# gfxdisp/ColorVideoVDP

Measured on AMD Instinct MI355X. Metric: Mpixels/s, higher is better.
Workload: dtype f32; 1 GPU; 3840x2160 60fps, standard_4k, f32 input resident in HBM, 64-frame clip pair; frames_total=64, frames_this_gpu=64, input_dtype=f32, heatmap=none, frame_generator=cpu, block_frames=64, fused_levels=3

## Files before the change

### colorvideovdp_amd/_capi.py

```python
import ctypes as C
import os

MAX_FILTER_LEN = 65
MAX_LEVELS = 16
MAX_WINDOW = 256
CSF_NODES = 32
PROF_N = 6
PROF_NAMES = ("photometry", "temporal_fir", "pyr_reduce", "band_level0", "band_rest", "heatmap")
ABI_VERSION = 14
RESIZE_MODES = {"nearest": 0, "bilinear": 1, "bicubic": 2, "area": 3}

U8, U16, F16, F32, F32_DKL, YUV8, YUV16 = range(7)
HEATMAP = {None: 0, "none": 0, "raw": 1, "threshold": 2, "supra-threshold": 3}
BUF_HIST, BUF_GPYR, BUF_DDUMP, BUF_HEAT, BUF_Q, BUF_HSTATS, BUF_HCURVE = range(7)


class Params(C.Structure):
    _fields_ = [
        ("eotf", C.c_int32),
        ("Y_peak", C.c_float), ("Y_black", C.c_float), ("Y_refl", C.c_float), ("exposure", C.c_float),
        ("gamma", C.c_float),
        ("rgb2dkl", C.c_float * 9),
        ("mask_p", C.c_float),
        ("mask_c10", C.c_float),
        ("mask_q", C.c_float * 4),
        ("xcm", C.c_float * 16),
        ("ch_gain", C.c_float * 4),
        ("d_max10", C.c_float),
        ("sens_mul", C.c_float),
        ("blur_radius", C.c_int32),
        ("blur_taps", C.c_float * 13),
        ("beta", C.c_float), ("beta_t", C.c_float), ("beta_tch", C.c_float), ("beta_sch", C.c_float),
        ("jod_a", C.c_float), ("jod_exp", C.c_float), ("image_int", C.c_float),
        ("ch_w", C.c_float * 4),
        ("baseband_weight", C.c_float * 4),
        ("csf_logL_first", C.c_float), ("csf_logL_last", C.c_float),
    ]


class Clip(C.Structure):
    _fields_ = [
        ("batch", C.c_int32), ("channels", C.c_int32),
        ("height", C.c_int32), ("width", C.c_int32),
        ("is_video", C.c_int32),
        ("n_frames", C.c_int32),
        ("first_frame", C.c_int32),
        ("n_levels", C.c_int32),
        ("filter_len", C.c_int32),
        ("block_frames", C.c_int32),
        ("heatmap", C.c_int32),
        ("debug_dump", C.c_int32),
        ("raw_halo", C.c_int32), ("total_frames", C.c_int32),
        ("feature_size", C.c_int32), ("fuse_mode", C.c_int32), ("band_layout", C.c_int32),
        ("defer_bands", C.c_int32), ("score_frames", C.c_int32),
        ("taps", C.c_float * (4 * MAX_FILTER_LEN)),
        ("csf_rows", C.c_float * (MAX_LEVELS * 4 * CSF_NODES)),
    ]


class YuvFormat(C.Structure):
    _fields_ = [
        ("chroma", C.c_int32), ("bit_depth", C.c_int32), ("matrix", C.c_int32), ("reserved", C.c_int32),
        ("frame_stride_test", C.c_int64), ("frame_stride_ref", C.c_int64),
    ]


PSNR_AS_IS, PSNR_PU21, PSNR_Y, PSNR_RGB2020 = range(4)


class PsnrArgs(C.Structure):
    _fields_ = [
        ("target", C.c_int32), ("reserved", C.c_int32),
        ("pu_p", C.c_float * 7),
        ("pu_L_min", C.c_float), ("pu_L_max", C.c_float),
        ("pu_norm", C.c_float),
        ("rows", C.c_float * 9),
    ]


SSIM_WIN = 11


class SsimArgs(C.Structure):
    _fields_ = [
        ("target", C.c_int32), ("reserved", C.c_int32),
        ("win", C.c_float * SSIM_WIN),
        ("C1", C.c_float), ("C2", C.c_float),
        ("luma", C.c_float * 3),
        ("pu_p", C.c_float * 7),
        ("pu_L_min", C.c_float), ("pu_L_max", C.c_float),
        ("pu_norm", C.c_float),
    ]


MSSSIM_LEVELS = 5


class MsssimArgs(C.Structure):
    _fields_ = [
        ("ssim", SsimArgs),
        ("weights", C.c_float * MSSSIM_LEVELS),
        ("reserved", C.c_int32),
    ]


PREVIEW_AS_IS, PREVIEW_LINEAR, PREVIEW_PQ = range(3)
PREVIEW_F32, PREVIEW_RGBE, PREVIEW_RGB48 = range(3)
# ... 156 lines not shown
```

### colorvideovdp_amd/csrc/core.cpp

```cpp
#include <algorithm>
#include <cmath>
#include <cstdarg>
#include <cstdio>
#include <cstdlib>
#include <cstring>
#include <string>
#include <vector>

#include "kernels.h"

using namespace cvvdp;

namespace {

struct Level {
  int H = 0, W = 0;
  int64_t P = 0;
  size_t g_off = 0, heat_off = 0, dd_off = 0, fd_off = 0, fs_off = 0;
  bool split_edge = false;
  bool feat4 = false;
  int f_pieces = 0;
  size_t partial_off = 0;
  int n_strip = 1, n_seg = 1, seg_h = 1;
  bool blur = false;
// ... 77 lines not shown
  return CVVDP_OK;
}

void join_pipeline(cvvdp_handle* h, hipStream_t s) {
  for (int i = 0; i < 2; ++i) {
    if (h->band_pending[i]) {
      (void)hipStreamWaitEvent(s, h->ev_band[i], 0);
      h->band_pending[i] = false;
    }
  }
}

struct ProfScope {
  cvvdp_handle* h; hipStream_t s; ProfEvent* ev = nullptr;
  ProfScope(cvvdp_handle* h_, int cat, hipStream_t s_) : h(h_), s(s_) {
    if (!h->prof) return;
    if (h->events_used == h->events.size()) {
      ProfEvent e{};
      if (hipEventCreate(&e.a) != hipSuccess || hipEventCreate(&e.b) != hipSuccess) return;
      h->events.push_back(e);
    }
    ev = &h->events[h->events_used++];
    ev->cat = cat;
    (void)hipEventRecord(ev->a, s);
  }
  ~ProfScope() { if (ev) (void)hipEventRecord(ev->b, s); }
};

constexpr float kGaussK0 = (float)(0.25 - 0.4 / 2.0);

void fill_csf(const cvvdp_handle* h, int level, float* lut) {
  std::memcpy(lut, h->c.csf_rows + (size_t)level * 4 * CVVDP_CSF_NODES, sizeof(float) * 4 * CVVDP_CSF_NODES);
}

void heat_weights(const cvvdp_handle* h, bool baseband, float* w) {
  const float t_int = h->c.is_video ? 1.0f : h->p.image_int;
  for (int c = 0; c < 4; ++c) {
    w[c] = h->p.ch_w[c] * t_int;
    if (baseband) w[c] = w[c] * h->p.baseband_weight[c];
  }
}

int run_bands(cvvdp_handle* h, int n_frames, int q_frame_offset, int set, hipStream_t s, int l_begin = 0, int l_end = -1, bool fused = false, int item0 = 0);

int run_pyramid_and_bands(cvvdp_handle* h, int n_frames, int q_frame_offset, hipStream_t s, int item0 = 0) {
  const int B = h->c.batch, items = n_frames * B, L = h->L, nch = h->nch;
  const float K[5] = {kGaussK0, 0.25f, 0.4f, 0.25f, kGaussK0};
  const int set = h->pipeline ? h->cur_set : 0;
  static const bool fuse2 = dev_knob("CVVDP_REDUCE2", 1) != 0;
  const int F = h->pipeline ? 0 : h->fuse_levels;
  if (F > 0) {
    if (int e = run_bands(h, n_frames, q_frame_offset, 0, s, 0, F, true, item0)) return e;
  }
  for (int l = F; l + 1 < L; ++l) {
    ProfScope ps(h, CVVDP_PROF_REDUCE, s);
    if (fuse2 && l + 2 < L && reduce2_supported(h->lv[l].H, h->lv[l].W)) {
      Reduce2Args r{};
      r.in = gbase(h, l, set) + (l == 0 ? (size_t)item0 * h->lv[0].P : 0); r.out1 = gbase(h, l + 1, set); r.out2 = gbase(h, l + 2, set);
      r.H = h->lv[l].H; r.W = h->lv[l].W; r.H1 = h->lv[l + 1].H; r.W1 = h->lv[l + 1].W; r.H2 = h->lv[l + 2].H; r.W2 = h->lv[l + 2].W;
      r.n_img = items; r.img_cap = level_cap(h, l); r.img_cap_out = h->items_cap_s; r.n_planes = 2 * nch;
      for (int i = 0; i < 5; ++i) r.k[i] = K[i];
      launch_reduce2(r, s);
      ++l;
      continue;
    }
    ReduceArgs r{};
    r.in = gbase(h, l, set) + (l == 0 ? (size_t)item0 * h->lv[0].P : 0);
    r.out = gbase(h, l + 1, set);
    r.H = h->lv[l].H; r.W = h->lv[l].W; r.Ho = h->lv[l + 1].H; r.Wo = h->lv[l + 1].W;
    r.n_img = items; r.img_cap = level_cap(h, l); r.img_cap_out = h->items_cap_s; r.n_planes = 2 * nch;
    for (int i = 0; i < 5; ++i) r.k[i] = K[i];
    launch_reduce(r, s);
  }
  if (int e = check_launch(h, "reduce")) return e;
  if (!h->pipeline) return run_bands(h, n_frames, q_frame_offset, 0, s, F, -1, false, item0);
  if (int e = ensure_pipeline_objects(h)) return e;
  (void)hipEventRecord(h->ev_reduce[set], s);
  (void)hipStreamWaitEvent(h->band_stream, h->ev_reduce[set], 0);
  if (int e = run_bands(h, n_frames, q_frame_offset, set, h->band_stream)) return e;
  (void)hipEventRecord(h->ev_band[set], h->band_stream);
  h->band_pending[set] = true;
  h->cur_set ^= 1;
  return CVVDP_OK;
}

int run_bands(cvvdp_handle* h, int n_frames, int q_frame_offset, int set, hipStream_t s, int l_begin, int l_end, bool fused, int item0) {
  const int B = h->c.batch, items = n_frames * B, L = h->L, nch = h->nch;
  if (l_begin == 0) h->last_range_done = false;
  if (l_end < 0) l_end = L - 1;
  const float K[5] = {kGaussK0, 0.25f, 0.4f, 0.25f, kGaussK0};
  const bool heat = h->c.heatmap != CVVDP_HEATMAP_NONE;
  static const bool fork_env = dev_knob("CVVDP_BAND_STREAMS", 1) != 0;
  static const int fork_max = dev_knob("CVVDP_BAND_STREAMS_MAX", 1024);
  static const int fork_tail = dev_knob("CVVDP_BAND_STREAMS_TAIL", 1);
  const int l_size = (fork_tail && !fused) ? std::min(l_begin, L - 1) : 0;
  bool fork = !fused && fork_env && L - l_size >= 4 && (int64_t)items * h->lv[l_size].n_strip * h->lv[l_size].n_seg <= fork_max;
  if (fork && !h->aux_stream[0]) {
    bool ok = hipEventCreateWithFlags(&h->ev_fork, hipEventDisableTiming) == hipSuccess;
    for (int i = 0; i < 2 && ok; ++i)
      ok = hipStreamCreateWithFlags(&h->aux_stream[i], hipStreamNonBlocking) == hipSuccess &&
           hipEventCreateWithFlags(&h->ev_join[i], hipEventDisableTiming) == hipSuccess;
    if (!ok) return fail(h, CVVDP_E_HIP, "cannot create the side streams of the band stage");
  }
  if (fork) {
    (void)hipEventRecord(h->ev_fork, s);
    for (int i = 0; i < 2; ++i) (void)hipStreamWaitEvent(h->aux_stream[i], h->ev_fork, 0);
  }
  hipStream_t const s_main = s;
// ... 160 lines not shown
    if (h->edge_stream[i]) { (void)hipStreamSynchronize(h->edge_stream[i]); (void)hipStreamDestroy(h->edge_stream[i]); }
    if (h->ev_edge_fork[i]) (void)hipEventDestroy(h->ev_edge_fork[i]);
    if (h->ev_edge_join[i]) (void)hipEventDestroy(h->ev_edge_join[i]);
  }
  delete h;
}

const char* cvvdp_last_error(const cvvdp_handle* h) { return h ? t_err.c_str() : "null handle"; }
int cvvdp_build_flags(void) {
  int f = tu_flags_band4() | tu_flags_band4f() | tu_flags_band4s();
#ifdef CVVDP_DEV_KNOBS
  f |= CVVDP_BUILD_DEV_KNOBS;
#endif
  return f;
}

#define CVVDP_STR2(x) #x
#define CVVDP_STR(x) CVVDP_STR2(x)
const char* cvvdp_build_info(void) {
#ifdef __clang_version__
#define CVVDP_COMPILER "clang " __clang_version__
#else
#define CVVDP_COMPILER "host compiler " __VERSION__
#endif
  return CVVDP_COMPILER "; HIP " CVVDP_STR(HIP_VERSION_MAJOR) "." CVVDP_STR(HIP_VERSION_MINOR) "." CVVDP_STR(HIP_VERSION_PATCH) "; gfx950";
}
int cvvdp_compiled_hip_version(void) { return HIP_VERSION; }
int cvvdp_runtime_hip_version(void) {
  int v = 0;
  if (hipRuntimeGetVersion(&v) != hipSuccess) return 0;
  return v;
}

int cvvdp_configure(cvvdp_handle* h, const cvvdp_clip* clip) {
  if (!h || !clip) return CVVDP_E_ARG;
  if (h->band_stream && (h->band_pending[0] || h->band_pending[1])) {
    (void)hipStreamSynchronize(h->band_stream);
    h->band_pending[0] = h->band_pending[1] = false;
  }
  const cvvdp_clip& c = *clip;
  if (c.batch < 1 || c.height < 2 || c.width < 2 || c.n_frames < 1) return fail(h, CVVDP_E_ARG, "bad clip geometry");
  if (c.channels != 1 && c.channels != 3) return fail(h, CVVDP_E_ARG, "channels must be 1 or 3");
  if (c.n_levels < 1 || c.n_levels > CVVDP_MAX_LEVELS) return fail(h, CVVDP_E_ARG, "n_levels out of range");
  if (c.is_video) {
    if (c.filter_len < 1 || c.filter_len > CVVDP_MAX_FILTER_LEN) return fail(h, CVVDP_E_UNSUPPORTED, "filter_len %d unsupported (max %d)", c.filter_len, CVVDP_MAX_FILTER_LEN);
    if (c.block_frames < 1 || c.filter_len - 1 + c.block_frames > CVVDP_MAX_WINDOW) return fail(h, CVVDP_E_ARG, "block_frames out of range");
  }
  if (c.heatmap != CVVDP_HEATMAP_NONE && c.batch != 1) return fail(h, CVVDP_E_UNSUPPORTED, "heat maps need batch == 1");
  if (c.feature_size < 0) return fail(h, CVVDP_E_ARG, "feature_size must be >= 0");
  if (c.feature_size > 0 && (c.heatmap != CVVDP_HEATMAP_NONE || c.debug_dump))
    return fail(h, CVVDP_E_UNSUPPORTED, "feature_size > 0 cannot be combined with a heat map or debug_dump");
  if (c.fuse_mode < 0 || c.fuse_mode > 2) return fail(h, CVVDP_E_ARG, "fuse_mode must be 0, 1 or 2");
  if (c.band_layout < 0 || c.band_layout > 1) return fail(h, CVVDP_E_ARG, "band_layout must be 0 or 1");
  if (c.defer_bands < 0 || c.defer_bands > 1) return fail(h, CVVDP_E_ARG, "defer_bands must be 0 or 1");
  if (c.defer_bands) {
    if (!c.is_video) return fail(h, CVVDP_E_ARG, "defer_bands is for video clips");
    if (c.score_frames < 1 || c.score_frames > c.block_frames) return fail(h, CVVDP_E_ARG, "score_frames must be in 1 .. block_frames");
    if (c.debug_dump || c.feature_size > 0) return fail(h, CVVDP_E_UNSUPPORTED, "defer_bands cannot be combined with debug_dump or features");
  }
  h->c = c;
  h->nch = c.is_video ? 4 : 3;
  h->L = c.n_levels;
  h->items_cap = (c.is_video ? c.block_frames : 1) * c.batch;
  h->items_cap_s = c.defer_bands ? c.score_frames * c.batch : h->items_cap;
  h->filtered_frames = 0;
  h->lv.assign(h->L, Level());
  int H = c.height, W = c.width;
  const int pad = h->p.blur_radius;
  for (int l = 0; l < h->L; ++l) {
    Level& lv = h->lv[l];
    lv.H = H; lv.W = W; lv.P = (int64_t)H * W;
    lv.blur = pad > 0 && H > pad && W > pad;
    lv.vec4 = lv.blur && W >= 16 && H >= 16;
    lv.feat4 = c.feature_size > 0 && lv.vec4 && l + 1 < h->L;
    const int sw = lv.vec4 ? kBand4StripWidth : (lv.blur ? 256 - 2 * pad : 256);
    lv.n_strip = (W + sw - 1) / sw;
    {
      const int clip_frames = c.total_frames > 0 ? c.total_frames : 64;
      static const int target_env = dev_knob("CVVDP_SEG_TARGET", 0);
      static const int rows_env = dev_knob("CVVDP_SEG_ROWS", 0);
      const int nominal = c.is_video ? std::min(c.heatmap != CVVDP_HEATMAP_NONE ? 16 : 64, clip_frames) : 1, target = target_env > 0 ? target_env : 768;
      const int max_rows = rows_env > 0 ? rows_env : (c.is_video ? 384 : 256);
      const int per_seg = lv.n_strip * nominal * c.batch;
      const int want = (target + per_seg - 1) / per_seg;
      const int lo = (H + max_rows - 1) / max_rows, hi = std::max(lo, (H + 15) / 16);
      lv.n_seg = std::min(std::max(want, lo), hi);
      lv.seg_h = (H + lv.n_seg - 1) / lv.n_seg;
      lv.seg_h += lv.seg_h & 1;
      lv.n_seg = (H + lv.seg_h - 1) / lv.seg_h;
      const int n_edge = lv.vec4 ? band4_edge_strips(W, lv.n_strip) : 0;
      lv.split_edge = n_edge > 0 && n_edge < lv.n_strip && (int64_t)(lv.n_strip - n_edge) * lv.n_seg * nominal * c.batch >= 1536;
    }
    if (l + 1 < h->L && (H < 2 || W < 2)) return fail(h, CVVDP_E_ARG, "pyramid too deep for %dx%d", c.width, c.height);
    H = (H + 1) / 2; W = (W + 1) / 2;
  }
  if (pad != 0 && pad != 6) return fail(h, CVVDP_E_UNSUPPORTED, "blur radius %d unsupported", pad);
  h->fuse_levels = 0;
  {
    const int clip_frames = c.total_frames > 0 ? c.total_frames : 64;
    const int nominal = c.is_video ? std::min(64, clip_frames) : 1;
    static const int fuse_max = dev_knob("CVVDP_FUSE_LEVELS", CVVDP_MAX_LEVELS);
    const bool plain = c.is_video && !c.debug_dump;
    const bool big = (int64_t)nominal * c.batch * h->lv[0].n_strip * h->lv[0].n_seg > 1024;
    if (plain && c.fuse_mode != 2 && (big || c.fuse_mode == 1))
      while (h->fuse_levels < fuse_max && h->fuse_levels + 1 < h->L && h->lv[h->fuse_levels].vec4 &&
             band4f_supported(h->lv[h->fuse_levels].H, h->lv[h->fuse_levels].W) &&
// ... 940 lines not shown
```

### colorvideovdp_amd/csrc/kernels.h

```cpp
#pragma once
#include <hip/hip_runtime.h>
#include <stdint.h>
#include "../../include/cvvdp_hip.h"

namespace cvvdp {

constexpr float kEps = 0.00001f;

#ifdef CVVDP_DEV_KNOBS
inline int dev_knob(const char* name, int dflt) { const char* v = getenv(name); return v ? atoi(v) : dflt; }
#else
constexpr int dev_knob(const char*, int dflt) { return dflt; }
#endif

#ifdef __HIPCC__
__device__ __forceinline__ float fast_log2(float x) { return __builtin_amdgcn_logf(x); }
__device__ __forceinline__ float fast_exp2(float x) { return __builtin_amdgcn_exp2f(x); }
__device__ __forceinline__ float fast_rcp(float x) { return __builtin_amdgcn_rcpf(x); }
__device__ __forceinline__ float fast_pow(float x, float p) { return fast_exp2(p * fast_log2(x)); }

__device__ __forceinline__ float expand_even(float m0, float m1, float m2, float e0, float e1) {
  return __builtin_fmaf(m2, e0, __builtin_fmaf(m1, e1, m0 * e0));
}
__device__ __forceinline__ float expand_odd(float m1, float m2, float eo) { return __builtin_fmaf(m2, eo, m1 * eo); }
// ... 56 lines not shown
void launch_resize(const ResizeArgs& a, hipStream_t s);
struct FirArgs {
  const void* src[2];
  int64_t sb[2], sc[2], sf[2], sh[2], sw[2];
  int32_t dtype;
  DisplayArgs dm;
  int32_t W, P, batch, n_frames, fl;
  int32_t raw_first;
  int32_t abs_first;
  int32_t write_hist;
  int32_t halo_run;
  float* hist;
  int64_t h_side, h_plane, h_slot, h_b;
  float* out;
  int64_t o_plane;
  float taps[4 * CVVDP_MAX_FILTER_LEN];
  float taps_rot[4 * CVVDP_ROT_TAPS];
  YuvArgs yuv;
  int16_t hist_src[CVVDP_MAX_FILTER_LEN];
};
static_assert(sizeof(FirArgs) <= 4096, "kernel arguments of the temporal kernels");
void launch_fir(const FirArgs& a, float* hist_shadow, hipStream_t s);
inline bool fir_has_register_window(int fl) { return fl == 7 || fl == 9 || fl == 13 || fl == 15 || fl == 17 || fl == 25 || fl == 31; }
inline int fir_kernel_len(int fl) {
  const int have[] = {7, 9, 13, 15, 17, 25, 31};
  for (int k : have) if (fl > 1 && fl <= k) return k;
  return fl;
}

struct ResampleArgs {
  FirArgs f;
  int32_t n_src[2];
  int32_t n_out, depth;
  const float* weights[2];
  const int32_t* emit[2];
  float* out[2];
};
static_assert(sizeof(ResampleArgs) <= 4096, "kernel arguments of the resampling temporal kernel");
inline bool fir_resampled_has_window(int depth) { return depth == 8 || depth == 12 || depth == 18 || depth == 26; }
void launch_fir_resampled(const ResampleArgs& a, bool generic, hipStream_t s);
int fir_resampled_prepare(cvvdp_handle* h, const void* t, const void* r, const cvvdp_yuv_format* fmt, int32_t H, int32_t W,
                          const int32_t n_src[2], int32_t depth, const float* w_t, const float* w_r, const int32_t* e_t, const int32_t* e_r,
                          int32_t n_out, float* out_t, float* out_r, ResampleArgs& a);
int fir_resampled_check_launch(cvvdp_handle* h);

struct ReduceArgs {
  const float* in;
  float* out;
  int32_t H, W, Ho, Wo, n_img;
  int32_t img_cap;
  int32_t img_cap_out;
  int32_t n_planes;
  float k[5];
};
void launch_reduce(const ReduceArgs& a, hipStream_t s);
struct Reduce2Args {
  const float* in;
  float *out1, *out2;
  int32_t H, W, H1, W1, H2, W2, n_img, img_cap, img_cap_out, n_planes;
  int32_t seg2;
  float k[5];
};
bool reduce2_supported(int H, int W);
constexpr int64_t kReduceRefPixels = 16384;
bool reduce_takes_ref_kernel(int H, int W);
void launch_reduce2(const Reduce2Args& a, hipStream_t s);

struct BandArgs {
  const float* g;
  const float* gc;
  int32_t H, W, Hc, Wc;
  int32_t items, items_cap, items_cap_c, nch;
  int32_t seg_h, n_seg, n_strip;
  int32_t per_xcd;
  int32_t strip0, n_strip_l;
  float band_mul;
  float lut[4 * CVVDP_CSF_NODES];
  float logL_first, logL_last;
  float sens_mul;
  float ch_gain[4];
  float mask_c10, mask_p, eps_p;
  float q[4], eps_q[4];
  float xw[16];
  float dmax;
  float m1[4];
  float inv_dmax;
  float blur_h[13];
  float ind_k1, ind_k0;
  float blur[13];
  float kx[3];
  float* partial;
  float* dchr;
  uint32_t* hstats;
  float hw[4];
  float beta_tch, eps_btch, eps_inv_btch;
  float* ddump;
  float* fdump;
  float* fsum;
  int32_t fs, f_pieces;
  float* g1_out;
  float rk[5];
  int32_t one_wave_layout;
};
void launch_band(const BandArgs& a, bool blur, hipStream_t s);
void launch_band4(const BandArgs& a, bool split_edge, hipStream_t s, hipStream_t s_edge);
int band4_edge_strips(int W, int n_strip);
// ... 395 lines not shown
```

### colorvideovdp_amd/csrc/pyramid.hip

```cpp
#include <algorithm>
#include <cstdlib>
#include <type_traits>
#include "kernels.h"

namespace cvvdp {

constexpr int RT = 32;
constexpr int RIN = 2 * RT + 3;

__device__ __forceinline__ float dot5(float a0, float a1, float a2, float a3, float a4, float k0, float k1, float k2, float k3, float k4) {
  return __builtin_fmaf(a4, k4, __builtin_fmaf(a3, k3, __builtin_fmaf(a2, k2, __builtin_fmaf(a1, k1, a0 * k0))));
}
__device__ __forceinline__ float dot2(float a0, float a1, float k0, float k1) { return __builtin_fmaf(a1, k1, a0 * k0); }
__device__ __forceinline__ float mul_rn(float a, float b) {
#pragma clang fp contract(off)
  return a * b;
}
__device__ __forceinline__ float add_rn(float a, float b) {
#pragma clang fp contract(off)
  return a + b;
}
__device__ __forceinline__ float edge2_rn(float v, float x0, float k0, float x1, float k1) { return add_rn(v, add_rn(mul_rn(x0, k0), mul_rn(x1, k1))); }

__global__ __launch_bounds__(256) void k_reduce(ReduceArgs a) {
  __shared__ float s_in[RIN][RIN + 1];
  __shared__ float s_v[RT][RIN + 1];
  const int img = blockIdx.z;
  const int plane = img / a.n_img, it = img - plane * a.n_img;
  const float* in = a.in + ((int64_t)plane * a.img_cap + it) * a.H * a.W;
  float* out = a.out + ((int64_t)plane * a.img_cap_out + it) * a.Ho * a.Wo;
  const int oy0 = blockIdx.y * RT, ox0 = blockIdx.x * RT;
  const int iy0 = 2 * oy0 - 2, ix0 = 2 * ox0 - 2;
  const int t = threadIdx.x;
  for (int e = t; e < RIN * RIN; e += 256) {
    const int r = e / RIN, c = e - r * RIN;
    const int y = iy0 + r, x = ix0 + c;
    s_in[r][c] = (y >= 0 && y < a.H && x >= 0 && x < a.W) ? in[(int64_t)y * a.W + x] : 0.0f;
  }
  __syncthreads();
  const float k0 = a.k[0], k1 = a.k[1], k2 = a.k[2], k3 = a.k[3], k4 = a.k[4];
  for (int e = t; e < RT * RIN; e += 256) {
    const int r = e / RIN, c = e - r * RIN;
    const int oy = oy0 + r;
    float v = 0.0f;
    if (oy < a.Ho && ix0 + c >= 0 && ix0 + c < a.W) {
      const int pr = 2 * r;
      v = dot5(s_in[pr][c], s_in[pr + 1][c], s_in[pr + 2][c], s_in[pr + 3][c], s_in[pr + 4][c], k0, k1, k2, k3, k4);
      if (oy == 0) v = edge2_rn(v, s_in[0 - iy0][c], k1, s_in[1 - iy0][c], k0);
      if (oy == a.Ho - 1) {
        if (a.H & 1) v = edge2_rn(v, s_in[a.H - 1 - iy0][c], k3, s_in[a.H - 2 - iy0][c], k4);
        else v = add_rn(v, mul_rn(s_in[a.H - 1 - iy0][c], k4));
      }
    }
    s_v[r][c] = v;
  }
  __syncthreads();
  for (int e = t; e < RT * RT; e += 256) {
    const int r = e / RT, c = e - r * RT;
    const int oy = oy0 + r, ox = ox0 + c;
    if (oy >= a.Ho || ox >= a.Wo) continue;
    const int pc = 2 * c;
    float v = dot5(s_v[r][pc], s_v[r][pc + 1], s_v[r][pc + 2], s_v[r][pc + 3], s_v[r][pc + 4], k0, k1, k2, k3, k4);
    if (ox == 0) v = edge2_rn(v, s_v[r][0 - ix0], k1, s_v[r][1 - ix0], k0);
    if (ox == a.Wo - 1) {
      if (a.H & 1) v = edge2_rn(v, s_v[r][a.W - 1 - ix0], k3, s_v[r][a.W - 2 - ix0], k4);
      else v = add_rn(v, mul_rn(s_v[r][a.W - 1 - ix0], k4));
    }
    out[(int64_t)oy * a.Wo + ox] = v;
  }
}

constexpr int RSEG = 32;
typedef float v4f_ __attribute__((ext_vector_type(4)));

template <bool EDGE>
__device__ __forceinline__ void hreduce_row(const ReduceArgs& a, const float* img, int y, float live, int ox, bool first, bool last, float (&h)[4]) {
  const int ix = 2 * ox - 4;
  const float* row = img + (int64_t)min(max(y, 0), a.H - 1) * a.W;
  const float my = (y >= 0 && y < a.H) ? live : 0.0f;
  float v[16];
#pragma unroll
  for (int q = 0; q < 4; ++q) {
    const int x = ix + 4 * q;
    float4 t;
    if constexpr (EDGE) {
      t = *reinterpret_cast<const float4*>(row + min(max(x, 0), a.W - 4));
      const float mx = (x >= 0 && x < a.W) ? 1.0f : 0.0f;
      t.x *= mx; t.y *= mx; t.z *= mx; t.w *= mx;
    } else {
#ifdef R2_NT_LOADS
      const v4f_ q4 = __builtin_nontemporal_load(reinterpret_cast<const v4f_*>(row + x));
      t = make_float4(q4.x, q4.y, q4.z, q4.w);
#else
      t = *reinterpret_cast<const float4*>(row + x);
#endif
    }
    v[4 * q] = t.x; v[4 * q + 1] = t.y; v[4 * q + 2] = t.z; v[4 * q + 3] = t.w;
  }
  const float k0 = a.k[0] * my, k1 = a.k[1] * my, k2 = a.k[2] * my, k3 = a.k[3] * my, k4 = a.k[4] * my;
#pragma unroll
  for (int j = 0; j < 4; ++j) {
    h[j] = dot5(v[2 * j + 2], v[2 * j + 3], v[2 * j + 4], v[2 * j + 5], v[2 * j + 6], k0, k1, k2, k3, k4);
  }
  if constexpr (EDGE) {
    if (first) h[0] += dot2(v[4], v[5], k1, k0);
    if (last) {
      const int c1 = a.W - 1 - ix, c2 = a.W - 2 - ix;
      if (a.H & 1) h[3] += dot2(v[c1], v[c2], k3, k4);
      else h[3] = __builtin_fmaf(v[c1], k4, h[3]);
    }
  }
}

struct __attribute__((packed, aligned(4))) f4u { float x, y, z, w; };

__device__ __forceinline__ void hreduce_row_any(const ReduceArgs& a, const float* img, int y, int ox, float (&h)[4]) {
  const int ix = 2 * ox - 4;
  const float* row = img + (int64_t)min(max(y, 0), a.H - 1) * a.W;
  const float my = (y >= 0 && y < a.H) ? 1.0f : 0.0f;
  float v[16];
#pragma unroll
// ... 207 lines not shown
      for (int j = 0; j < 2; ++j) { w2[0][j] = w2[2][j]; w2[1][j] = w2[3][j]; w2[2][j] = w2[4][j]; }
    }
    l1row(2 * r2 + 1, w2[3]);
    l1row(2 * r2 + 2, w2[4]);
    float o2[2];
#pragma unroll
    for (int j = 0; j < 2; ++j) o2[j] = dot5(w2[0][j], w2[1][j], w2[2][j], w2[3][j], w2[4][j], k0, k1, k2, k3, k4);
    if (r2 == 0) {
#pragma unroll
      for (int j = 0; j < 2; ++j) o2[j] += dot2(w2[2][j], w2[3][j], k1, k0);
    }
    if (r2 == a.H2 - 1) {
      if (a.H1 & 1) {
#pragma unroll
        for (int j = 0; j < 2; ++j) o2[j] += dot2(w2[2][j], w2[1][j], k3, k4);
      } else {
#pragma unroll
        for (int j = 0; j < 2; ++j) o2[j] = __builtin_fmaf(w2[3][j], k4, o2[j]);
      }
    }
    if constexpr (ANYW) {
      if (own) {
        float* dst = out2 + (int64_t)r2 * a.W2 + 2 * v;
        if (2 * v < a.W2) dst[0] = o2[0];
        if (2 * v + 1 < a.W2) dst[1] = o2[1];
      }
    } else {
      if (own) *reinterpret_cast<float2*>(out2 + (int64_t)r2 * a.W2 + 2 * v) = make_float2(o2[0], o2[1]);
    }
  }
}

bool reduce2_supported(int H, int W) {
  return (W % 16 == 0 || W >= 32) && H >= 8 && !reduce_takes_ref_kernel(H, W) && !reduce_takes_ref_kernel((H + 1) / 2, (W + 1) / 2);
}

void launch_reduce2(const Reduce2Args& a0, hipStream_t s) {
  Reduce2Args a = a0;
  const bool anyw = a.W % 16 != 0;
  const int nq = (a.W1 + 3) / 4, waves = (nq + R2_LANES - 1) / R2_LANES, bx = (waves + 3) / 4;
  static const int seg_cap = std::max(4, dev_knob("CVVDP_R2_SEG", R2_SEG));
  int n_seg = (a.H2 + seg_cap - 1) / seg_cap;
  const int64_t per_seg = (int64_t)bx * a.n_planes * a.n_img;
  n_seg = (int)std::max<int64_t>(n_seg, std::min<int64_t>((4096 + per_seg - 1) / per_seg, (a.H2 + 15) / 16));
  a.seg2 = (a.H2 + n_seg - 1) / n_seg;
  dim3 grid(bx, (a.H2 + a.seg2 - 1) / a.seg2, a.n_planes * a.n_img);
  if (anyw) hipLaunchKernelGGL(k_reduce2<true>, grid, dim3(256), 0, s, a);
  else hipLaunchKernelGGL(k_reduce2<false>, grid, dim3(256), 0, s, a);
}

bool reduce_takes_ref_kernel(int H, int W) { return (int64_t)H * W <= kReduceRefPixels || W < 16 || H < 4; }

void launch_reduce(const ReduceArgs& a, hipStream_t s) {
  if (reduce_takes_ref_kernel(a.H, a.W)) {
    dim3 grid((a.Wo + RT - 1) / RT, (a.Ho + RT - 1) / RT, a.n_planes * a.n_img);
    hipLaunchKernelGGL(k_reduce, grid, dim3(256), 0, s, a);
    return;
  }
  if (a.W % 8 == 0 && a.H >= 4) {
    dim3 grid((a.Wo / 4 + 255) / 256, (a.Ho + RSEG - 1) / RSEG, a.n_planes * a.n_img);
    hipLaunchKernelGGL(k_reduce_vec<false>, grid, dim3(256), 0, s, a);
    return;
  }
  if (a.W >= 16 && a.H >= 4) {
    dim3 grid(((a.Wo + 3) / 4 + 255) / 256, (a.Ho + RSEG - 1) / RSEG, a.n_planes * a.n_img);
    hipLaunchKernelGGL(k_reduce_vec<true>, grid, dim3(256), 0, s, a);
    return;
  }
  dim3 grid((a.Wo + RT - 1) / RT, (a.Ho + RT - 1) / RT, a.n_planes * a.n_img);
  hipLaunchKernelGGL(k_reduce, grid, dim3(256), 0, s, a);
}

__global__ __launch_bounds__(256) void k_expand_add(ExpandAddArgs a) {
  const int pix = blockIdx.x * 256 + threadIdx.x;
  if (pix >= a.H * a.W) return;
  const int img = blockIdx.y;
  const float* c = a.coarse + (int64_t)img * a.Hc * a.Wc;
  float* f = a.fine + (int64_t)img * a.H * a.W;
  const int y = pix / a.W, x = pix - y * a.W;
  const int my = y >> 1, mx = x >> 1;
  const int y0 = max(my - 1, 0), y2 = min(my + 1, a.Hc - 1);
  const int x0 = max(mx - 1, 0), x2 = min(mx + 1, a.Wc - 1);
  const float e0 = a.kx[0], e1 = a.kx[1], o = a.kx[2];
  auto vert = [&](int cx) -> float {
    if (y & 1) return expand_odd(c[(int64_t)my * a.Wc + cx], c[(int64_t)y2 * a.Wc + cx], o);
    return expand_even(c[(int64_t)y0 * a.Wc + cx], c[(int64_t)my * a.Wc + cx], c[(int64_t)y2 * a.Wc + cx], e0, e1);
  };
  float v;
  if (x & 1) v = expand_odd(vert(mx), vert(x2), o);
  else v = expand_even(vert(x0), vert(mx), vert(x2), e0, e1);
  f[pix] += v;
}

__global__ __launch_bounds__(256) void k_expand_add4(ExpandAddArgs a) {
  const int wq = a.W >> 2;
  const int q = blockIdx.x * 256 + threadIdx.x;
  if (q >= a.H * wq) return;
  const int img = blockIdx.y;
  const float* c = a.coarse + (int64_t)img * a.Hc * a.Wc;
  float* f = a.fine + (int64_t)img * a.H * a.W;
  const int y = q / wq, x = (q - y * wq) << 2;
  const int my = y >> 1, mx = x >> 1;
  const int y0 = max(my - 1, 0), y2 = min(my + 1, a.Hc - 1);
  const float e0 = a.kx[0], e1 = a.kx[1], o = a.kx[2];
  float v[4];
#pragma unroll
// ... 85 lines not shown
```

### colorvideovdp_amd/cvvdp_metric.py

```python
import collections
import concurrent.futures
import ctypes
import json
import math
import time

import numpy as np
import torch

from . import _capi
from . import host_setup as hs
from ._frames import batch_strides, yuv_block_resized
from .config import config_files, json2dict, load_config
from .display_model import vvdp_display_geometry, vvdp_display_photo_eotf, vvdp_display_photometry
from .sharding import all_gather_frames, plan_frame_shard
from .video_source import reshuffle_dims, video_source, video_source_array
from .vq_metric import register_metric, vq_exception, vq_metric

f32 = np.float32


def _storage_is_unshared(t):
    try:
        return torch._C._storage_Use_Count(t.untyped_storage()._cdata) <= 2
# ... 185 lines not shown
    def finish(self):
        self._deliver()


class _JodLoss(torch.autograd.Function):

    @staticmethod
    def forward(ctx, test, reference, metric, dim_order):
        jod, grad = metric.predict_with_gradient(test, reference, dim_order)
        ctx.save_for_backward(grad)
        ctx.batch_shape = [n if ch == "B" else 1 for ch, n in zip(dim_order.upper(), grad.shape)]
        return 10.0 - jod

    @staticmethod
    def backward(ctx, upstream):
        grad, = ctx.saved_tensors
        up = upstream if upstream.dim() == 0 else upstream.reshape(ctx.batch_shape)
        return -grad * up, None, None, None


class cvvdp(vq_metric):
    def __init__(self, display_name="standard_4k", display_photometry=None, display_geometry=None, config_paths=[],
                 heatmap=None, quiet=False, device=None, temp_padding="replicate", use_checkpoints=False, dump_channels=None,
                 gpu_mem=None, block_frames=None):
        self.quiet = quiet
        self.heatmap = heatmap
        self.temp_padding = temp_padding
        self.use_checkpoints = use_checkpoints
        self.gpu_mem = gpu_mem
        self.block_frames = block_frames
        self.training_mode = False
        assert heatmap in ["threshold", "supra-threshold", "raw", "none", None], "Unknown heatmap type"
        self.do_heatmap = (self.heatmap is not None) and (self.heatmap != "none")
        if dump_channels is not None and not all(hasattr(dump_channels, a) for a in ("open", "enabled", "writer")):
            raise vq_exception("dump_channels must be a colorvideovdp_amd.dump_channels.DumpChannels")
        self.dump_channels = dump_channels
        _capi.lib()
        if device is None:
            self.device = torch.device("cuda")
        else:
            self.device = torch.device(device)
        if self.device.type != "cuda":
            raise RuntimeError("colorvideovdp_amd runs on an MI355X only: device must be a CUDA/HIP device; there is no CPU path")
        if self.device.index is None and torch.cuda.is_available():
            self.device = torch.device("cuda", torch.cuda.current_device())
        self._cfg_version = 0
        self._handle = ctypes.c_void_p()
        self._ws = None
        self._shard = None
        self.debug_dump = False
        self.score_frames = None
        self.band_layout = 0
        self.fuse_mode = 0
        self.set_display_model(display_name, display_photometry=display_photometry, display_geometry=display_geometry,
                               config_paths=config_paths)
        self.load_config(config_paths)

    def __del__(self):
        try:
            if getattr(self, "_handle", None) is not None and self._handle.value:
                _capi.lib().cvvdp_destroy(self._handle)
                self._handle = ctypes.c_void_p()
        except Exception:
            pass

    _INT_PARAMETERS = ("pu_dilate", "filter_len")
    _LIST_LENGTHS = {"mask_q": 4, "xcm_weights": 16, "baseband_weight": 4, "sigma_tf": 4, "beta_tf": 4}

    def _param_device(self):
        return self.device if torch.cuda.is_available() else torch.device("cpu")

    def __getattr__(self, name):
        p = self.__dict__.get("parameters")
        if p is not None and name in p and not isinstance(p[name], (str, bool)):
            return torch.as_tensor(p[name], dtype=torch.float32 if isinstance(p[name], (float, list)) else None, device=self._param_device())
        raise AttributeError(f"'{type(self).__name__}' object has no attribute '{name}'")

    def __setattr__(self, name, value):
        p = self.__dict__.get("parameters")
        if p is not None and name in p and name != "filter_len" and not isinstance(p[name], (str, bool)):
            q = dict(p)
            q[name] = self._parameter_value(name, value, p[name])
            self._set_parameters(q)
            return
        object.__setattr__(self, name, value)

    @classmethod
    def _parameter_value(cls, name, value, current):
        v = value.detach().to("cpu", torch.float32) if torch.is_tensor(value) else torch.as_tensor(np.asarray(value), dtype=torch.float32)
        if isinstance(current, list):
            if v.dim() != 1 or v.numel() != len(current):
                raise ValueError(f"parameter '{name}' holds {len(current)} values, got shape {tuple(v.shape)}")
            return [float(x) for x in v.tolist()]
        if v.numel() != 1:
            raise ValueError(f"parameter '{name}' is a scalar, got shape {tuple(v.shape)}")
        x = float(v.reshape(()).item())
        if name in cls._INT_PARAMETERS:
            if x != round(x):
                raise ValueError(f"parameter '{name}' is an integer, got {x}")
            return int(round(x))
        return x

    def train(self, do_training=True):
        self.training_mode = do_training

    def load_config(self, config_paths):
# ... 358 lines not shown
    def _upload_frames(self, x, a, b):
        if x.device == self.device:
            return x[:, :, a:b]
        if x.device.type != "cpu" or (a == 0 and b == x.shape[2]) or not x.is_contiguous():
            return x[:, :, a:b].to(self.device, non_blocking=True)
        out = torch.empty((x.shape[0], x.shape[1], b - a) + tuple(x.shape[3:]), dtype=x.dtype, device=self.device)
        for i in range(x.shape[0]):
            for c in range(x.shape[1]):
                out[i, c].copy_(x[i, c, a:b], non_blocking=True)
        return out

    @staticmethod
    def _host_resident(vs):
        if hasattr(vs, "get_raw_yuv_block"):
            return not getattr(vs, "device_resident", False)
        if isinstance(vs, video_source_array):
            return vs.raw_arrays()[0].device.type == "cpu"
        if hasattr(vs, "get_raw_block"):
            return not getattr(vs, "device_resident", True)
        return False

    _strides = staticmethod(batch_strides)

    def _route(self, vs, first):
        height, width, n_total = vs.get_video_size()
        is_image = n_total == 1
        pyr_height, freqs = hs.band_frequencies(width, height, self.pix_per_deg)
        L = pyr_height + 1
        rho_band = freqs.copy()
        rho_band[L - 1] = 0.1
        is_yuv = hasattr(vs, "get_raw_yuv_block")
        yuv_resized = is_yuv and bool(getattr(vs, "needs_resize", lambda: False)())
        generic = not self._is_raw_source(vs)
        prefiltered = bool(getattr(vs, "is_temporally_filtered", False)) and not is_image
        if prefiltered and not generic:
            raise vq_exception("is_temporally_filtered is only meaningful for sources that deliver 'DKLd65_trans' frames")
        self._seq = None
        probe_t = probe_r = code = None
        if is_yuv:
            if is_image:
                raise vq_exception("single-frame .yuv clips are not supported")
            C = 3
        elif generic and not is_image:
            C, code = 3, _capi.F32_DKL
        else:
            probe_t, probe_r, code = self._raw_block(vs, first, first + 1)
            C = probe_t.shape[1]
        return _Route(height, width, n_total, vs.get_batch_size(), L, rho_band, is_image, is_yuv, yuv_resized, generic, prefiltered,
                      3 if is_image else 4, C, code, probe_t, probe_r)

    def _plan_clip(self, vs, rt, first, count):
        height, width, is_image, prefiltered = rt.height, rt.width, rt.is_image, rt.prefiltered
        key = (height, width, rt.n_total, first, count, rt.B, rt.C, is_image, None if is_image else float(vs.get_frames_per_second()), self.heatmap,
               bool(self.debug_dump or self.dump_channels is not None), int(self.fuse_mode), int(self.band_layout), self.score_frames, self._sink_on_device, self.block_frames, self.gpu_mem, float(self.pix_per_deg), self._cfg_version, prefiltered, getattr(self, "_feature_out", None) is not None,
               self._host_resident(vs))
        cached = getattr(self, "_clip_cache", None)
        if cached is not None and cached[0] == key:
            clip, fl, F = cached[1], cached[2], cached[3]
            if not is_image:
                self.F, self.filter_len, self.last_block_frames = F, fl, clip.block_frames
            return clip, fl, F
        clip = _capi.Clip()
        clip.batch, clip.channels, clip.height, clip.width = rt.B, rt.C, height, width
        clip.is_video, clip.n_frames, clip.n_levels = int(not is_image), count, rt.L
        clip.first_frame = first
        clip.total_frames = rt.n_total
        clip.heatmap = _capi.HEATMAP[self.heatmap]
        clip.debug_dump = int(bool(self.debug_dump or self.dump_channels is not None))
        clip.fuse_mode = int(self.fuse_mode)
        clip.band_layout = int(self.band_layout)
        clip.feature_size = int(math.ceil(self.pix_per_deg)) if getattr(self, "_feature_out", None) is not None else 0
        clip.raw_halo = int(not is_image and not self._host_resident(vs) and (rt.is_yuv or isinstance(vs, video_source_array) or hasattr(vs, "get_raw_block")))
        fl, F = 1, None
        if not is_image:
            F = hs.temporal_filters(vs.get_frames_per_second(), self.parameters["beta_tf"], self.parameters["sigma_tf"])
            self.F = F
            fl = 1 if prefiltered else F.shape[1]
            if fl > _capi.MAX_FILTER_LEN:
                raise vq_exception(f"frame rates above {(_capi.MAX_FILTER_LEN - 1) * 4} fps are not supported")
            self.filter_len = fl
            taps = np.zeros((4, _capi.MAX_FILTER_LEN), dtype=f32)
            taps[:, :fl] = F[:, :fl]
            clip.taps[:] = taps.reshape(-1).tolist()
            nb = self._pick_block_frames(height * width, rt.B, count, fl, rt.nch, self._host_resident(vs), bool(clip.raw_halo))
            clip.filter_len, clip.block_frames = fl, nb
            self.last_block_frames = nb
            piece = self._piece_frames()
            if self.do_heatmap and clip.raw_halo and not prefiltered and not clip.debug_dump and nb > piece:
                clip.defer_bands, clip.score_frames = 1, piece
        rows = np.zeros((_capi.MAX_LEVELS, 4, _capi.CSF_NODES), dtype=f32)
        for bb in range(rt.L):
            rows[bb] = self.csf_table.rows(rt.rho_band[bb])
        clip.csf_rows[:] = rows.reshape(-1).tolist()
        self._clip_cache = (key, clip, fl, F)
        return clip, fl, F

    def _bind_workspace(self, clip, is_image):
        lib = _capi.lib()
        while True:
            _capi.check(self._handle, lib.cvvdp_configure(self._handle, ctypes.byref(clip)), "cvvdp_configure")
            need = lib.cvvdp_workspace_bytes(self._handle)
            if self._ws is not None and self._ws.numel() >= need and self._ws.device == self.device:
                break
            self._ws = None
            try:
                self._ws = self._alloc_workspace(need)
                break
            except torch.cuda.OutOfMemoryError:
                nb_now = int(clip.block_frames)
                if is_image or self.block_frames is not None or nb_now <= 1:
                    raise
                torch.cuda.empty_cache()
                clip.block_frames = 64 if nb_now > 64 else max(1, nb_now // 2)
                self.last_block_frames = int(clip.block_frames)
                if clip.defer_bands and clip.block_frames <= clip.score_frames:
                    clip.defer_bands, clip.score_frames = 0, 0
        _capi.check(self._handle, lib.cvvdp_bind_workspace(self._handle, self._ws.data_ptr(), self._ws.numel()), "cvvdp_bind_workspace")
        self.last_score_frames = int(clip.score_frames) if clip.defer_bands else 0

    def _alloc_features(self, rt, clip, count):
        if getattr(self, "_feature_out", None) is None:
            return
        fs = int(clip.feature_size)
# ... 262 lines not shown
```

### include/cvvdp_hip.h

```cpp
#ifndef CVVDP_HIP_H
#define CVVDP_HIP_H

#include <stddef.h>
#include <stdint.h>

#ifdef __cplusplus
extern "C" {
#endif

#define CVVDP_ABI_VERSION 14
#define CVVDP_MAX_FILTER_LEN 65
#define CVVDP_MAX_LEVELS 16
#define CVVDP_MAX_WINDOW 256
#define CVVDP_CSF_NODES 32

enum {
  CVVDP_OK = 0,
  CVVDP_E_ARG = -1,
  CVVDP_E_STATE = -2,
  CVVDP_E_HIP = -3,
  CVVDP_E_UNSUPPORTED = -4
};

enum { CVVDP_U8 = 0, CVVDP_U16 = 1, CVVDP_F16 = 2, CVVDP_F32 = 3, CVVDP_F32_DKL = 4 ,
       CVVDP_YUV8 = 5, CVVDP_YUV16 = 6 };
enum { CVVDP_EOTF_SRGB = 0, CVVDP_EOTF_PQ = 1, CVVDP_EOTF_HLG = 2, CVVDP_EOTF_LINEAR = 3, CVVDP_EOTF_GAMMA = 4 };
enum { CVVDP_HEATMAP_NONE = 0, CVVDP_HEATMAP_RAW = 1, CVVDP_HEATMAP_THRESHOLD = 2, CVVDP_HEATMAP_SUPRA = 3 };
enum { CVVDP_BUF_HIST = 0, CVVDP_BUF_GPYR = 1, CVVDP_BUF_DDUMP = 2, CVVDP_BUF_HEAT = 3, CVVDP_BUF_Q = 4, CVVDP_BUF_HSTATS = 5, CVVDP_BUF_HCURVE = 6 };

typedef struct cvvdp_params {
  int32_t eotf;
  float Y_peak, Y_black, Y_refl, exposure;
  float gamma;
  float rgb2dkl[9];
  float mask_p;
  float mask_c10;
  float mask_q[4];
  float xcm[16];
  float ch_gain[4];
  float d_max10;
  float sens_mul;
  int32_t blur_radius;
  float blur_taps[13];
  float beta, beta_t, beta_tch, beta_sch;
  float jod_a, jod_exp, image_int;
  float ch_w[4];
  float baseband_weight[4];
  float csf_logL_first, csf_logL_last;
} cvvdp_params;

typedef struct cvvdp_clip {
  int32_t batch, channels;
  int32_t height, width;
  int32_t is_video;
  int32_t n_frames;
  int32_t first_frame;
  int32_t n_levels;
  int32_t filter_len;
  int32_t block_frames;
  int32_t heatmap;
  int32_t debug_dump;
  int32_t raw_halo;
  int32_t total_frames;
  int32_t feature_size;
  int32_t fuse_mode;
  int32_t band_layout;
  int32_t defer_bands;
  int32_t score_frames;
  float taps[4 * CVVDP_MAX_FILTER_LEN];
  float csf_rows[CVVDP_MAX_LEVELS * 4 * CVVDP_CSF_NODES];
} cvvdp_clip;

typedef struct cvvdp_handle cvvdp_handle;

int cvvdp_abi_version(void);
#define CVVDP_BUILD_DEV_KNOBS 1
#define CVVDP_BUILD_SAFE_LOADS 2
#define CVVDP_BUILD_DIAG 4
int cvvdp_build_flags(void);
const char* cvvdp_build_info(void);
int cvvdp_compiled_hip_version(void);
int cvvdp_runtime_hip_version(void);
void cvvdp_struct_sizes(int32_t* params_bytes, int32_t* clip_bytes);

int cvvdp_create(const cvvdp_params* params, cvvdp_handle** out);
void cvvdp_destroy(cvvdp_handle* h);
const char* cvvdp_last_error(const cvvdp_handle* h);

int cvvdp_configure(cvvdp_handle* h, const cvvdp_clip* clip);
size_t cvvdp_workspace_bytes(const cvvdp_handle* h);
int cvvdp_fused_levels(const cvvdp_handle* h);
int cvvdp_bind_workspace(cvvdp_handle* h, void* dev_workspace, size_t bytes);

int cvvdp_put_image(cvvdp_handle* h, const void* dev_test, const void* dev_ref, int32_t dtype,
                    const int64_t strides_test[5], const int64_t strides_ref[5], void* stream);

int cvvdp_process_block(cvvdp_handle* h, const void* dev_test, const void* dev_ref, int32_t dtype,
                        const int64_t strides_test[5], const int64_t strides_ref[5], int32_t raw_first,
                        const int32_t* hist_src, int32_t n_frames, int32_t q_frame_offset, void* stream);

typedef struct cvvdp_yuv_format {
  int32_t chroma;
  int32_t bit_depth;
  int32_t matrix;
  int32_t reserved;
  int64_t frame_stride_test, frame_stride_ref;
} cvvdp_yuv_format;
int cvvdp_process_block_yuv(cvvdp_handle* h, const void* dev_test, const void* dev_ref, const cvvdp_yuv_format* fmt,
                            int32_t raw_first, const int32_t* hist_src, int32_t n_frames, int32_t q_frame_offset,
                            void* stream);

enum { CVVDP_RESIZE_NEAREST = 0, CVVDP_RESIZE_BILINEAR = 1, CVVDP_RESIZE_BICUBIC = 2, CVVDP_RESIZE_AREA = 3 };
int cvvdp_unpack_yuv_resized(cvvdp_handle* h, const void* dev_codes, const cvvdp_yuv_format* fmt, int32_t is_ref, int32_t src_width,
                             int32_t src_height, int32_t n_frames, int32_t dst_width, int32_t dst_height, int32_t mode, float* dev_tmp,
                             float* dev_rgb, void* stream);

int cvvdp_fir_resampled_yuv(cvvdp_handle* h, const void* dev_test, const void* dev_ref, const cvvdp_yuv_format* fmt, int32_t height,
                            int32_t width, const int32_t n_src[2], int32_t depth, const float* dev_weights_test,
                            const float* dev_weights_ref, const int32_t* dev_emit_test, const int32_t* dev_emit_ref, int32_t n_out,
                            int32_t generic, float* dev_out_test, float* dev_out_ref, void* stream);

// ... 145 lines not shown
```

Before: 37120 Mpixel/s.

## Chain small pyramid reduce levels into one per-image kernel launch

Once a pyramid level is small enough to use the reference reduce kernel, all remaining reduce levels are computed in a single launch. One 1024-thread block per image plane loops over tiles and levels, reading each level's output from global memory as the next level's input. This removes a series of small kernel launches for the tail levels. In exchange, each image gets only one workgroup for the tail, so parallelism is lower. A new tail_route field is added to the clip struct and ABI, and defaults to the chained path.

```diff
diff --git a/colorvideovdp_amd/_capi.py b/colorvideovdp_amd/_capi.py
--- a/colorvideovdp_amd/_capi.py
+++ b/colorvideovdp_amd/_capi.py
@@ -52,7 +52,7 @@
         ("debug_dump", C.c_int32),
         ("raw_halo", C.c_int32), ("total_frames", C.c_int32),
         ("feature_size", C.c_int32), ("fuse_mode", C.c_int32), ("band_layout", C.c_int32),
-        ("defer_bands", C.c_int32), ("score_frames", C.c_int32),
+        ("defer_bands", C.c_int32), ("score_frames", C.c_int32), ("tail_route", C.c_int32),
         ("taps", C.c_float * (4 * MAX_FILTER_LEN)),
         ("csf_rows", C.c_float * (MAX_LEVELS * 4 * CSF_NODES)),
     ]
diff --git a/colorvideovdp_amd/csrc/core.cpp b/colorvideovdp_amd/csrc/core.cpp
--- a/colorvideovdp_amd/csrc/core.cpp
+++ b/colorvideovdp_amd/csrc/core.cpp
@@ -153,8 +153,21 @@
   if (F > 0) {
     if (int e = run_bands(h, n_frames, q_frame_offset, 0, s, 0, F, true, item0)) return e;
   }
+  const bool chain = h->c.tail_route == 0;
   for (int l = F; l + 1 < L; ++l) {
     ProfScope ps(h, CVVDP_PROF_REDUCE, s);
+    if (chain && l + 2 < L && reduce_takes_ref_kernel(h->lv[l].H, h->lv[l].W)) {
+      ReduceArgs r{};
+      r.in = gbase(h, l, set) + (l == 0 ? (size_t)item0 * h->lv[0].P : 0);
+      r.out = gbase(h, l + 1, set);
+      r.H = h->lv[l].H; r.W = h->lv[l].W; r.Ho = h->lv[l + 1].H; r.Wo = h->lv[l + 1].W;
+      r.n_img = items; r.img_cap = level_cap(h, l); r.img_cap_out = h->items_cap_s; r.n_planes = 2 * nch;
+      for (int i = 0; i < 5; ++i) r.k[i] = K[i];
+      r.n_more = L - 2 - l;
+      for (int j = 0; j < r.n_more; ++j) r.more_out[j] = gbase(h, l + 2 + j, set);
+      launch_reduce(r, s);
+      break;
+    }
     if (fuse2 && l + 2 < L && reduce2_supported(h->lv[l].H, h->lv[l].W)) {
       Reduce2Args r{};
       r.in = gbase(h, l, set) + (l == 0 ? (size_t)item0 * h->lv[0].P : 0); r.out1 = gbase(h, l + 1, set); r.out2 = gbase(h, l + 2, set);
@@ -421,6 +434,7 @@
     return fail(h, CVVDP_E_UNSUPPORTED, "feature_size > 0 cannot be combined with a heat map or debug_dump");
   if (c.fuse_mode < 0 || c.fuse_mode > 2) return fail(h, CVVDP_E_ARG, "fuse_mode must be 0, 1 or 2");
   if (c.band_layout < 0 || c.band_layout > 1) return fail(h, CVVDP_E_ARG, "band_layout must be 0 or 1");
+  if (c.tail_route < 0 || c.tail_route > 1) return fail(h, CVVDP_E_ARG, "tail_route must be 0 or 1");
   if (c.defer_bands < 0 || c.defer_bands > 1) return fail(h, CVVDP_E_ARG, "defer_bands must be 0 or 1");
   if (c.defer_bands) {
     if (!c.is_video) return fail(h, CVVDP_E_ARG, "defer_bands is for video clips");
diff --git a/colorvideovdp_amd/csrc/kernels.h b/colorvideovdp_amd/csrc/kernels.h
--- a/colorvideovdp_amd/csrc/kernels.h
+++ b/colorvideovdp_amd/csrc/kernels.h
@@ -132,6 +132,8 @@
   int32_t img_cap_out;
   int32_t n_planes;
   float k[5];
+  int32_t n_more;
+  float* more_out[CVVDP_MAX_LEVELS - 2];
 };
 void launch_reduce(const ReduceArgs& a, hipStream_t s);
 struct Reduce2Args {
diff --git a/colorvideovdp_amd/csrc/pyramid.hip b/colorvideovdp_amd/csrc/pyramid.hip
--- a/colorvideovdp_amd/csrc/pyramid.hip
+++ b/colorvideovdp_amd/csrc/pyramid.hip
@@ -22,25 +22,22 @@
 }
 __device__ __forceinline__ float edge2_rn(float v, float x0, float k0, float x1, float k1) { return add_rn(v, add_rn(mul_rn(x0, k0), mul_rn(x1, k1))); }
 
-__global__ __launch_bounds__(256) void k_reduce(ReduceArgs a) {
-  __shared__ float s_in[RIN][RIN + 1];
-  __shared__ float s_v[RT][RIN + 1];
-  const int img = blockIdx.z;
-  const int plane = img / a.n_img, it = img - plane * a.n_img;
-  const float* in = a.in + ((int64_t)plane * a.img_cap + it) * a.H * a.W;
-  float* out = a.out + ((int64_t)plane * a.img_cap_out + it) * a.Ho * a.Wo;
-  const int oy0 = blockIdx.y * RT, ox0 = blockIdx.x * RT;
+struct ReduceGeom { int32_t H, W, Ho, Wo; float k[5]; };
+template <bool TRIM, int NT>
+__device__ __forceinline__ void reduce_tile(const ReduceGeom& a, const float* in, float* out, int oy0, int ox0, float (&s_in)[RIN][RIN + 1], float (&s_v)[RT][RIN + 1]) {
   const int iy0 = 2 * oy0 - 2, ix0 = 2 * ox0 - 2;
   const int t = threadIdx.x;
-  for (int e = t; e < RIN * RIN; e += 256) {
-    const int r = e / RIN, c = e - r * RIN;
+  const int nr = TRIM ? min(RT, a.Ho - oy0) : RT, nc = TRIM ? min(RT, a.Wo - ox0) : RT;
+  const int pr_n = TRIM ? 2 * nr + 3 : RIN, pc_n = TRIM ? 2 * nc + 3 : RIN;
+  for (int e = t; e < pr_n * pc_n; e += NT) {
+    const int r = e / pc_n, c = e - r * pc_n;
     const int y = iy0 + r, x = ix0 + c;
     s_in[r][c] = (y >= 0 && y < a.H && x >= 0 && x < a.W) ? in[(int64_t)y * a.W + x] : 0.0f;
   }
   __syncthreads();
   const float k0 = a.k[0], k1 = a.k[1], k2 = a.k[2], k3 = a.k[3], k4 = a.k[4];
-  for (int e = t; e < RT * RIN; e += 256) {
-    const int r = e / RIN, c = e - r * RIN;
+  for (int e = t; e < nr * pc_n; e += NT) {
+    const int r = e / pc_n, c = e - r * pc_n;
     const int oy = oy0 + r;
     float v = 0.0f;
     if (oy < a.Ho && ix0 + c >= 0 && ix0 + c < a.W) {
@@ -55,8 +52,8 @@
     s_v[r][c] = v;
   }
   __syncthreads();
-  for (int e = t; e < RT * RT; e += 256) {
-    const int r = e / RT, c = e - r * RT;
+  for (int e = t; e < nr * nc; e += NT) {
+    const int r = e / nc, c = e - r * nc;
     const int oy = oy0 + r, ox = ox0 + c;
     if (oy >= a.Ho || ox >= a.Wo) continue;
     const int pc = 2 * c;
@@ -67,6 +64,44 @@
       else v = add_rn(v, mul_rn(s_v[r][a.W - 1 - ix0], k4));
     }
     out[(int64_t)oy * a.Wo + ox] = v;
+  }
+}
+
+__global__ __launch_bounds__(256) void k_reduce(ReduceArgs a) {
+  __shared__ float s_in[RIN][RIN + 1];
+  __shared__ float s_v[RT][RIN + 1];
+  const int img = blockIdx.z;
+  const int plane = img / a.n_img, it = img - plane * a.n_img;
+  const float* in = a.in + ((int64_t)plane * a.img_cap + it) * a.H * a.W;
+  float* out = a.out + ((int64_t)plane * a.img_cap_out + it) * a.Ho * a.Wo;
+  ReduceGeom g;
+  g.H = a.H; g.W = a.W; g.Ho = a.Ho; g.Wo = a.Wo;
+#pragma unroll
+  for (int i = 0; i < 5; ++i) g.k[i] = a.k[i];
+  reduce_tile<false, 256>(g, in, out, blockIdx.y * RT, blockIdx.x * RT, s_in, s_v);
+}
+
+constexpr int kChainThreads = 1024;
+__global__ __launch_bounds__(kChainThreads) void k_reduce_chain(ReduceArgs a) {
+  __shared__ float s_in[RIN][RIN + 1];
+  __shared__ float s_v[RT][RIN + 1];
+  const int img = blockIdx.x;
+  const int plane = img / a.n_img, it = img - plane * a.n_img;
+  const float* in = a.in + ((int64_t)plane * a.img_cap + it) * a.H * a.W;
+  ReduceGeom g;
+  g.Ho = a.H; g.Wo = a.W;
+#pragma unroll
+  for (int i = 0; i < 5; ++i) g.k[i] = a.k[i];
+  for (int j = 0; j <= a.n_more; ++j) {
+    g.H = g.Ho; g.W = g.Wo; g.Ho = (g.H + 1) >> 1; g.Wo = (g.W + 1) >> 1;
+    float* out = (j == 0 ? a.out : a.more_out[j - 1]) + ((int64_t)plane * a.img_cap_out + it) * g.Ho * g.Wo;
+    for (int oy0 = 0; oy0 < g.Ho; oy0 += RT) {
+      for (int ox0 = 0; ox0 < g.Wo; ox0 += RT) {
+        reduce_tile<true, kChainThreads>(g, in, out, oy0, ox0, s_in, s_v);
+        __syncthreads();
+      }
+    }
+    in = out;
   }
 }
 
@@ -380,6 +415,10 @@
 bool reduce_takes_ref_kernel(int H, int W) { return (int64_t)H * W <= kReduceRefPixels || W < 16 || H < 4; }
 
 void launch_reduce(const ReduceArgs& a, hipStream_t s) {
+  if (a.n_more > 0) {
+    hipLaunchKernelGGL(k_reduce_chain, dim3(a.n_planes * a.n_img), dim3(kChainThreads), 0, s, a);
+    return;
+  }
   if (reduce_takes_ref_kernel(a.H, a.W)) {
     dim3 grid((a.Wo + RT - 1) / RT, (a.Ho + RT - 1) / RT, a.n_planes * a.n_img);
     hipLaunchKernelGGL(k_reduce, grid, dim3(256), 0, s, a);
diff --git a/colorvideovdp_amd/cvvdp_metric.py b/colorvideovdp_amd/cvvdp_metric.py
--- a/colorvideovdp_amd/cvvdp_metric.py
+++ b/colorvideovdp_amd/cvvdp_metric.py
@@ -261,6 +261,7 @@
         self.score_frames = None
         self.band_layout = 0
         self.fuse_mode = 0
+        self.tail_route = 0
         self.set_display_model(display_name, display_photometry=display_photometry, display_geometry=display_geometry,
                                config_paths=config_paths)
         self.load_config(config_paths)
@@ -725,7 +726,7 @@
     def _plan_clip(self, vs, rt, first, count):
         height, width, is_image, prefiltered = rt.height, rt.width, rt.is_image, rt.prefiltered
         key = (height, width, rt.n_total, first, count, rt.B, rt.C, is_image, None if is_image else float(vs.get_frames_per_second()), self.heatmap,
-               bool(self.debug_dump or self.dump_channels is not None), int(self.fuse_mode), int(self.band_layout), self.score_frames, self._sink_on_device, self.block_frames, self.gpu_mem, float(self.pix_per_deg), self._cfg_version, prefiltered, getattr(self, "_feature_out", None) is not None,
+               bool(self.debug_dump or self.dump_channels is not None), int(self.fuse_mode), int(self.band_layout), int(self.tail_route), self.score_frames, self._sink_on_device, self.block_frames, self.gpu_mem, float(self.pix_per_deg), self._cfg_version, prefiltered, getattr(self, "_feature_out", None) is not None,
                self._host_resident(vs))
         cached = getattr(self, "_clip_cache", None)
         if cached is not None and cached[0] == key:
@@ -742,6 +743,7 @@
         clip.debug_dump = int(bool(self.debug_dump or self.dump_channels is not None))
         clip.fuse_mode = int(self.fuse_mode)
         clip.band_layout = int(self.band_layout)
+        clip.tail_route = int(self.tail_route)
         clip.feature_size = int(math.ceil(self.pix_per_deg)) if getattr(self, "_feature_out", None) is not None else 0
         clip.raw_halo = int(not is_image and not self._host_resident(vs) and (rt.is_yuv or isinstance(vs, video_source_array) or hasattr(vs, "get_raw_block")))
         fl, F = 1, None
diff --git a/include/cvvdp_hip.h b/include/cvvdp_hip.h
--- a/include/cvvdp_hip.h
+++ b/include/cvvdp_hip.h
@@ -67,6 +67,7 @@
   int32_t band_layout;
   int32_t defer_bands;
   int32_t score_frames;
+  int32_t tail_route;
   float taps[4 * CVVDP_MAX_FILTER_LEN];
   float csf_rows[CVVDP_MAX_LEVELS * 4 * CVVDP_CSF_NODES];
 } cvvdp_clip;
```

Result: slower. 36050 Mpixel/s (-2.9%).
